# GBATZOLIS/conditional_score_diffusion

Measured on AMD Instinct MI355X. Metric: images/sec for 1000-step PC sampling, ddpm_paired_SR3 score net of celebA_SR3_160 (BASELINE configs[1]), 160x160, higher is better.
Workload: dtype f16x3 (every operand carried as hi + lo fp16 = 22 significand bits, 3 MFMAs per product, f32 accumulate; f32-class: the per-op test tolerance is the f32 kernel's, network error 1.9e-6 vs the reference); 1 GPU; BASELINE configs[1]: celebA_SR3_160 (ddpm_paired_SR3, nf=96, ch_mult (1,1,2,2,3,3), attn 20/10/5), 1000-step PC (reverse_diffusion + langevin, snr 0.15), batch 64 per GPU, random-init weights, synthetic LR inputs; images_per_gpu=64, global_batch=64, noise=on-device Philox4x32-10, precision_mode=fp16x3

## Files before the change

### conditional_score_diffusion_amd/csrc/conv_pw16.hip

```cpp
#include <stdlib.h>
#include <string.h>

#include "common.h"

namespace csd {

typedef _Float16 half8_t __attribute__((ext_vector_type(8)));
typedef float floatx4 __attribute__((ext_vector_type(4)));
typedef float v4f_t __attribute__((ext_vector_type(4)));
typedef unsigned int uint4_t __attribute__((ext_vector_type(4)));

#define PW_THREADS 256
#define PW_NTL 6
#define PW_WSCALE 256.0f
#ifndef PW_DEPTH
#define PW_DEPTH 2
#endif

struct PwKArgs {
  ConvArgs a;
  int C0, C1, Cout;
  int npix;
  int hw;
  int ks;
  int ntiles;
};

__device__ __forceinline__ float4 pw_gload4(const float* p) {
  const v4f_t v = *(const __attribute__((address_space(1))) v4f_t*)(p);
  return make_float4(v.x, v.y, v.z, v.w);
}

template <int NS, int MTP, int OCC>
__global__ __launch_bounds__(PW_THREADS, OCC) void pw16_kernel(const float* __restrict__ g_src0,
                                                          const float* __restrict__ g_src1,
                                                          const char* __restrict__ g_wpack, const PwKArgs k) {
  extern __shared__ __attribute__((aligned(16))) char smem[];
  constexpr int WPIX = MTP * 16;
  constexpr int TPIX = 4 * WPIX;
  const int tid = threadIdx.x;
  const int lane = tid & 63;
  const int wave = tid >> 6;
  const int l16 = lane & 15;
  const int kq = lane >> 4;
  const int ng = blockIdx.y;
  const int Cin = k.C0 + k.C1;

  const int wbytes = k.ks * PW_NTL * NS * 1024;
  float* const lds_bias = reinterpret_cast<float*>(smem + wbytes);
  const int col_base = ng * (PW_NTL * 16) + kq * 4;

  const int nt_mine = (k.ntiles - (int)blockIdx.x + (int)gridDim.x - 1) / (int)gridDim.x;
  const int total = nt_mine * k.ks;
  const bool has_norm = k.a.nscale != nullptr;
  const bool has_res = k.a.res != nullptr;
  const bool has_act = k.a.act == CSD_ACT_SWISH;
  const int ntl = min(PW_NTL, (k.Cout - (int)blockIdx.y * (PW_NTL * 16) + 15) / 16);

  constexpr int D = MTP == 1 ? 4 : PW_DEPTH;
  float4 raw[D][MTP][2];
  constexpr bool PFN = MTP == 1;
  float4 nsc[PFN ? D : 1][MTP][2], nsh[PFN ? D : 1][MTP][2];
  floatx4 acc[MTP][PW_NTL];
#pragma unroll
  for (int j = 0; j < MTP; ++j)
#pragma unroll
    for (int nt = 0; nt < PW_NTL; ++nt) acc[j][nt] = floatx4{0.f, 0.f, 0.f, 0.f};

  int l_tile = blockIdx.x, l_kk = 0, l_it = 0;
  int c_tile = blockIdx.x, c_kk = 0;

  auto issue = [&](float4 (&dst)[MTP][2], float4 (&dsc)[MTP][2], float4 (&dsh)[MTP][2]) {
    if (l_it < total) {
      const int kb = l_kk * 32;
      const bool s1 = kb >= k.C0;
      const float* src = s1 ? g_src1 : g_src0;
      const int C = s1 ? k.C1 : k.C0;
      const int ch = (s1 ? kb - k.C0 : kb) + kq * 8;
#pragma unroll
      for (int j = 0; j < MTP; ++j) {
        int p = l_tile * TPIX + wave * WPIX + j * 16 + l16;
        p = p < k.npix ? p : k.npix - 1;
        const float* q = src + (size_t)p * C + ch;
        dst[j][0] = pw_gload4(q);
        dst[j][1] = pw_gload4(q + 4);
        if (PFN && has_norm) {
          const size_t row = (size_t)(p / k.hw) * Cin + l_kk * 32 + kq * 8;
          dsc[j][0] = pw_gload4(k.a.nscale + row); dsc[j][1] = pw_gload4(k.a.nscale + row + 4);
          dsh[j][0] = pw_gload4(k.a.nshift + row); dsh[j][1] = pw_gload4(k.a.nshift + row + 4);
        }
      }
      ++l_it;
      if (++l_kk == k.ks) { l_kk = 0; l_tile += gridDim.x; }
    }
  };

#pragma unroll
  for (int u = 0; u < D; ++u) issue(raw[u], nsc[PFN ? u : 0], nsh[PFN ? u : 0]);

  wg_copy_to_lds<PW_THREADS, 9>(smem, g_wpack + (size_t)ng * wbytes, wbytes, tid);
  if (tid < PW_NTL * 16) {
    const int c = ng * (PW_NTL * 16) + tid;
    lds_bias[tid] = (k.a.bias && c < k.Cout) ? k.a.bias[c] : 0.f;
  }
  __syncthreads();

  for (int it = 0; it < total; it += D) {
#pragma unroll
    for (int u = 0; u < D; ++u) {
      if (it + u < total) {
        half8_t bh[MTP], bl[MTP];
#pragma unroll
        for (int j = 0; j < MTP; ++j) {
          float v[8] = {raw[u][j][0].x, raw[u][j][0].y, raw[u][j][0].z, raw[u][j][0].w,
                        raw[u][j][1].x, raw[u][j][1].y, raw[u][j][1].z, raw[u][j][1].w};
          if (has_norm) {
            float4 s0, s1, h0, h1;
            if constexpr (PFN) {
              s0 = nsc[u][j][0]; s1 = nsc[u][j][1]; h0 = nsh[u][j][0]; h1 = nsh[u][j][1];
            } else {
              int p = c_tile * TPIX + wave * WPIX + j * 16 + l16;
              p = p < k.npix ? p : k.npix - 1;
              const size_t row = (size_t)(p / k.hw) * Cin + c_kk * 32 + kq * 8;
              s0 = pw_gload4(k.a.nscale + row); s1 = pw_gload4(k.a.nscale + row + 4);
              h0 = pw_gload4(k.a.nshift + row); h1 = pw_gload4(k.a.nshift + row + 4);
            }
            const float sc[8] = {s0.x, s0.y, s0.z, s0.w, s1.x, s1.y, s1.z, s1.w};
            const float sh[8] = {h0.x, h0.y, h0.z, h0.w, h1.x, h1.y, h1.z, h1.w};
#pragma unroll
            for (int q = 0; q < 8; ++q) v[q] = fmaf(v[q], sc[q], sh[q]);
            if (has_act) {
#pragma unroll
              for (int q = 0; q < 8; ++q) v[q] = v[q] * __builtin_amdgcn_rcpf(1.0f + __expf(-v[q]));
            }
          }
#pragma unroll
          for (int q = 0; q < 8; ++q) {
            const _Float16 hi = (_Float16)v[q];
            bh[j][q] = hi;
            if (NS == 2) bl[j][q] = (_Float16)(v[q] - (float)hi);
          }
        }
        issue(raw[u], nsc[PFN ? u : 0], nsh[PFN ? u : 0]);
        const char* wk = smem + (size_t)c_kk * PW_NTL * NS * 1024 + lane * 16;
#pragma unroll
        for (int nt = 0; nt < PW_NTL; ++nt) {
          if (nt >= ntl) continue;
          const half8_t wh = *reinterpret_cast<const half8_t*>(wk + (nt * NS) * 1024);
          half8_t wl;
          if (NS == 2) wl = *reinterpret_cast<const half8_t*>(wk + (nt * NS + 1) * 1024);
#pragma unroll
          for (int j = 0; j < MTP; ++j) {
            if (NS == 2) {
              acc[j][nt] = __builtin_amdgcn_mfma_f32_16x16x32_f16(wl, bh[j], acc[j][nt], 0, 0, 0);
              acc[j][nt] = __builtin_amdgcn_mfma_f32_16x16x32_f16(wh, bl[j], acc[j][nt], 0, 0, 0);
            }
            acc[j][nt] = __builtin_amdgcn_mfma_f32_16x16x32_f16(wh, bh[j], acc[j][nt], 0, 0, 0);
          }
        }
        if (++c_kk == k.ks) {
          constexpr unsigned OOB = 0x80000000u;
          constexpr int RSRC_FLAGS = 0x00020000;
          const size_t p_base = (size_t)c_tile * TPIX + wave * WPIX;
          const int left = k.npix - (int)p_base;
          const __amdgpu_buffer_rsrc_t out_r = __builtin_amdgcn_make_buffer_rsrc(
              k.a.out + p_base * k.a.out_stride + k.a.out_coff, 0, OOB, RSRC_FLAGS);
          const __amdgpu_buffer_rsrc_t res_r = __builtin_amdgcn_make_buffer_rsrc(
              const_cast<float*>(has_res ? k.a.res + p_base * k.Cout : k.a.out), 0, OOB, RSRC_FLAGS);
          const float unscale = 1.0f / PW_WSCALE;
#pragma unroll
          for (int j = 0; j < MTP; ++j) {
            const int pl = j * 16 + l16;
            const bool pv = pl < left;
            uint4_t rv[PW_NTL];
#pragma unroll
            for (int nt = 0; nt < PW_NTL; ++nt) {
              const int col0 = col_base + nt * 16;
              const unsigned off = (pv && has_res && col0 < k.Cout) ? (unsigned)(pl * k.Cout + col0) * 4u : OOB;
              rv[nt] = __builtin_amdgcn_raw_buffer_load_b128(res_r, off, 0, 0);
            }
#pragma unroll
            for (int nt = 0; nt < PW_NTL; ++nt) {
              const int col0 = col_base + nt * 16;
              const float4 b = *reinterpret_cast<const float4*>(lds_bias + nt * 16 + kq * 4);
              uint4_t ov;
              ov.x = __float_as_uint(((acc[j][nt][0] * unscale + b.x) + __uint_as_float(rv[nt].x)) * k.a.out_scale);
              ov.y = __float_as_uint(((acc[j][nt][1] * unscale + b.y) + __uint_as_float(rv[nt].y)) * k.a.out_scale);
              ov.z = __float_as_uint(((acc[j][nt][2] * unscale + b.z) + __uint_as_float(rv[nt].z)) * k.a.out_scale);
              ov.w = __float_as_uint(((acc[j][nt][3] * unscale + b.w) + __uint_as_float(rv[nt].w)) * k.a.out_scale);
              const unsigned off = (pv && col0 < k.Cout) ? (unsigned)(pl * k.a.out_stride + col0) * 4u : OOB;
              __builtin_amdgcn_raw_buffer_store_b128(ov, out_r, off, 0, 0);
              acc[j][nt] = floatx4{0.f, 0.f, 0.f, 0.f};
            }
          }
          c_kk = 0;
          c_tile += gridDim.x;
        }
      }
    }
  }
}

static size_t pw16_w_bytes(const ConvPlan& p, int ns) { return (size_t)((p.C0 + p.C1) / 32) * PW_NTL * ns * 1024; }
static size_t pw16_lds_bytes(const ConvPlan& p, int ns) { return pw16_w_bytes(p, ns) + PW_NTL * 16 * sizeof(float); }

bool pw16_supported(const ConvPlan& p, int ns) {
  return p.taps == 1 && p.stride == 1 && p.up == 0 && p.C0 > 0 && p.C0 % 32 == 0 && p.C1 % 32 == 0 && p.Cout % 4 == 0 &&
         (ns == 1 || ns == 2) && pw16_lds_bytes(p, ns) <= 150 * 1024;
}

size_t pw16_packed_bytes(const ConvPlan& p, int ns) {
  const int n_groups = cdiv(p.Cout, PW_NTL * 16);
  return (size_t)n_groups * pw16_w_bytes(p, ns);
}

__global__ void pw16_pack_kernel(const float* __restrict__ w, _Float16* __restrict__ wpack, int layout, int cin_src,
                                 int cout_src, int cout_off, int ks, int ns, int cout_pad) {
  const size_t idx = (size_t)blockIdx.x * blockDim.x + threadIdx.x;
  const int cin_tot = ks * 32;
  const int t_lo = cout_off / 16, t_hi = (cout_off + cout_src + 15) / 16;
  if (idx >= (size_t)(t_hi - t_lo) * 16 * cin_tot) return;
  const int cp = t_lo * 16 + (int)(idx / cin_tot);
  const int cin = (int)(idx % cin_tot);
  const int cout = cp - cout_off;
  if (cp >= cout_pad || cout < 0 || cout >= cout_src || cin >= cin_src) return;
  const float v = ((layout == 0) ? w[(size_t)cout * cin_src + cin] : w[(size_t)cin * cout_src + cout]) * PW_WSCALE;
  const int ng = cp / (PW_NTL * 16), nt = (cp % (PW_NTL * 16)) / 16, r = cp % 16;
  const int kk = cin / 32, kq = (cin % 32) / 8, q = cin % 8;
  const int lane = kq * 16 + r;
  _Float16* dst = wpack + ((((size_t)ng * ks + kk) * PW_NTL + nt) * ns) * 512 + lane * 8 + q;
  const _Float16 hi = (_Float16)v;
  dst[0] = hi;
  if (ns == 2) dst[512] = (_Float16)(v - (float)hi);
}

// ... 77 lines not shown
  const int y = ty0 + ty, x = tx0 + tx;
  if (y >= H || x >= W) return;
  float acc[CO];
#pragma unroll
  for (int c = 0; c < CO; ++c) acc[c] = 0.f;
#pragma unroll
  for (int tap = 0; tap < 9; ++tap) {
    const float* q = ts_tile + ((ty + tap / 3) * 18 + tx + tap % 3) * cp + tap * CO;
#pragma unroll
    for (int c = 0; c < CO; ++c) acc[c] += q[c];
  }
#pragma unroll
  for (int c = 0; c < CO; ++c) {
    const float r = ((acc[c] + bias[c]) + (res ? res[((b * H + y) * W + x) * CO + c] : 0.f)) * out_scale;
    if (nchw) out[((b * CO + c) * H + y) * W + x] = r;
    else out[((b * H + y) * W + x) * CO + c] = r;
  }
}

int tapsum_launch(const float* part, const float* bias, const float* res, float* out, int B, int H, int W, int cout, int nchw,
                  float out_scale, hipStream_t s) {
  const int cp = pw16_taps_cout(cout);
  const dim3 grid(cdiv(W, 16), cdiv(H, 16), B), block(256);
  const size_t lds = (size_t)324 * cp * sizeof(float);
  switch (cout) {
#define CSD_TS_CASE(CO)                                                                                                              \
  case CO: {                                                                                                                         \
    static bool attr_set = false;                                                                                                    \
    if (!attr_set && lds > 64 * 1024) {                               \
      CSD_CHECK_HIP(hipFuncSetAttribute(reinterpret_cast<const void*>(tapsum_kernel<CO>), hipFuncAttributeMaxDynamicSharedMemorySize, \
                                        160 * 1024));                                                                               \
      attr_set = true;                                                                                                               \
    }                                                                                                                                \
    hipLaunchKernelGGL(tapsum_kernel<CO>, grid, block, lds, s, part, bias, res, out, H, W, cp, nchw, out_scale);                     \
    break;                                                                                                                           \
  }
    CSD_TS_CASE(1) CSD_TS_CASE(2) CSD_TS_CASE(3) CSD_TS_CASE(4) CSD_TS_CASE(5) CSD_TS_CASE(6)
#undef CSD_TS_CASE
    default:
      set_error("tapsum: %d output channels not instantiated", cout);
      return CSD_ERR_INVALID;
  }
  CSD_LAUNCH_CHECK();
  return CSD_OK;
}

bool pw16_taps_supported(int cin, int cout, int ns) {
  ConvPlan p;
  memset(&p, 0, sizeof(p));
  p.taps = 1; p.stride = 1; p.C0 = cin; p.Cout = pw16_taps_cout(cout);
  return cout >= 1 && cout <= 6 && pw16_supported(p, ns) && !CSD_TUNE_ENV("CSD_NO_TAPSUM");
}

template <int NS, int MTP, int OCC>
static int pw16_launch_t(const PwKArgs& k, const ConvPlan& p, hipStream_t s) {
  auto kern = pw16_kernel<NS, MTP, OCC>;
  const size_t lds = pw16_lds_bytes(p, NS);
  static size_t attr_lds = 0;
  if (lds > attr_lds) {
    if (hipFuncSetAttribute(reinterpret_cast<const void*>(kern), hipFuncAttributeMaxDynamicSharedMemorySize, 160 * 1024) !=
        hipSuccess) {
      set_error("pw16: cannot raise the dynamic LDS limit");
      return CSD_ERR_HIP;
    }
    attr_lds = 160 * 1024;
  }
  const int n_groups = cdiv(p.Cout, PW_NTL * 16);
  int gx = (OCC * 256) / n_groups;
  if (gx < 1) gx = 1;
  if (gx > k.ntiles) gx = k.ntiles;
  hipLaunchKernelGGL(kern, dim3(gx, n_groups), dim3(PW_THREADS), lds, s, k.a.src0, k.a.src1,
                     reinterpret_cast<const char*>(k.a.wpack), k);
  CSD_LAUNCH_CHECK();
  return CSD_OK;
}

int pw16_launch(const ConvPlan& p, int ns, const ConvArgs& a, hipStream_t s) {
  CSD_REQUIRE(pw16_supported(p, ns), "pw16: unsupported layer (taps %d C0 %d C1 %d Cout %d)", p.taps, p.C0, p.C1, p.Cout);
  CSD_REQUIRE(!a.temb && !a.out_nchw && (a.act == CSD_ACT_NONE || (a.act == CSD_ACT_SWISH && a.nscale)),
              "pw16: temb / NCHW output / an activation without a GroupNorm are not supported");
  PwKArgs k;
  k.a = a;
  k.C0 = p.C0; k.C1 = p.C1; k.Cout = p.Cout;
  k.npix = p.B * p.OH * p.OW;
  k.hw = p.OH * p.OW;
  k.ks = (p.C0 + p.C1) / 32;
  const bool big = cdiv(k.npix, 128) >= 768;
  k.ntiles = cdiv(k.npix, big ? 128 : 64);
  if (ns == 2) return big ? pw16_launch_t<2, 2, 2>(k, p, s) : pw16_launch_t<2, 1, 2>(k, p, s);
  return big ? pw16_launch_t<1, 2, 3>(k, p, s) : pw16_launch_t<1, 1, 2>(k, p, s);
}

}
```

### conditional_score_diffusion_amd/csrc/conv_f16_q.hip

```cpp
#include <stdlib.h>
#include <type_traits>

#include "conv_f16_kernel.h"

namespace csd {

typedef float floatx4q __attribute__((ext_vector_type(4)));
typedef unsigned int uint4q __attribute__((ext_vector_type(4)));

#define C16Q_THREADS 256

__device__ __forceinline__ double dpp_row16_sum(double v) {
#define CSD_DPP_STEP(CTRL)                                                                                   \
  {                                                                                                          \
    const int lo = __builtin_amdgcn_mov_dpp(__double2loint(v), CTRL, 0xF, 0xF, true);                        \
    const int hi = __builtin_amdgcn_mov_dpp(__double2hiint(v), CTRL, 0xF, 0xF, true);                        \
    v += __hiloint2double(hi, lo);                                                                           \
  }
  CSD_DPP_STEP(0xB1)
  CSD_DPP_STEP(0x4E)
  CSD_DPP_STEP(0x124)
  CSD_DPP_STEP(0x128)
#undef CSD_DPP_STEP
  return v;
}
__device__ __forceinline__ float dpp_row16_sum(float v) {
#define CSD_DPP_STEP_F(CTRL) v += __int_as_float(__builtin_amdgcn_mov_dpp(__float_as_int(v), CTRL, 0xF, 0xF, true));
  CSD_DPP_STEP_F(0xB1)
  CSD_DPP_STEP_F(0x4E)
  CSD_DPP_STEP_F(0x124)
  CSD_DPP_STEP_F(0x128)
#undef CSD_DPP_STEP_F
  return v;
}

typedef int int8q __attribute__((ext_vector_type(8)));

template <int MQ, int NS, bool MASK, int PWC, int S, int NTQ, bool F8, bool UP4 = false, bool RAW = false>
__global__ __launch_bounds__(C16Q_THREADS, 2) void conv_f16_q_kernel(const void* __restrict__ g_hi,
                                                                    const void* __restrict__ g_lo,
                                                                    const char* __restrict__ g_wpack,
                                                                    const Conv16KArgs k) {
  static_assert(!UP4 || (S == 1 && !F8), "the phase form is the stride-1 Upsample conv (a resampling conv: full split)");
  static_assert(!RAW || (NS == 2 && !F8), "the fp32-source form splits into two fp16 planes");
  constexpr int TAPS = UP4 ? 4 : 9, KS = UP4 ? 2 : 3, KCS = 2;
  constexpr int LO = 32 * KCS;
  constexpr int PSB = 32 * KCS * NS + 16;
  constexpr int NPIX = 2 * MQ * 16;
  constexpr int SPP = 2 * NS * KCS;
  constexpr int NU0 = (S == 2) ? ((NS == 2) ? 10 : 5) : ((NS == 2) ? 7 : 4);
  constexpr int NU = RAW ? 2 * ((NU0 + 1) / 2) : NU0;
  constexpr int rstride = PWC * PSB;
  constexpr int WSTEP = NTQ * NS * 1024;
  constexpr int GC = 32 * NTQ, HC = 16 * NTQ;
  extern __shared__ __attribute__((aligned(16))) char smem16[];

  const int tid = threadIdx.x;
#ifdef CSD_C16_TIMING
  int ts_n = 0;
#define Q_TSTAMP() do { if (k.a.dbg && tid == 0 && blockIdx.x < 4095 && ts_n < 8) k.a.dbg[blockIdx.x * 8 + ts_n++] = clock64(); } while (0)
#else
#define Q_TSTAMP() do { } while (0)
#endif
  Q_TSTAMP();
  const int lane = tid & 63;
  const int wave = __builtin_amdgcn_readfirstlane(tid >> 6);
  const int mi = wave >> 1, ni = wave & 1;
  const int l16 = lane & 15, kq = lane >> 4;

  int w;
  {
    const int bid = blockIdx.x, nb = k.nblocks;
    const int xcd = bid & 7, slot = bid >> 3;
    const int q = nb >> 3, r = nb & 7;
    w = (xcd < r ? xcd * (q + 1) : r * (q + 1) + (xcd - r) * q) + slot;
  }
  const int ng = w % k.n_groups;
  const int tile4 = w / k.n_groups;
  const int ph = UP4 ? (tile4 & 3) : 0, pa = ph >> 1, pb = ph & 1;
  const int tile = UP4 ? (tile4 >> 2) : tile4;
  const int tile_y = tile / k.tiles_x;
  const int ov0 = tile_y * k.TH, ox0 = (tile - tile_y * k.tiles_x) * k.TW;
  const int Py = UP4 ? 1 - pa : ((S == 2) ? 0 : 1), Px = UP4 ? 1 - pb : ((S == 2) ? 0 : 1);
  const int prow0 = ov0 * S - Py, pcol0 = ox0 * S - Px;
  const int EH = (S == 2) ? k.IH : k.OH, EW = (S == 2) ? k.IW : k.OW;
  const int Cin = k.C0;
  const int npatch = k.PH * k.PW;
// ... 515 lines not shown
    CSD_CHECK_HIP(hipFuncSetAttribute(reinterpret_cast<const void*>(kern), hipFuncAttributeMaxDynamicSharedMemorySize, 160 * 1024));
    attr_set = true;
  }
  hipLaunchKernelGGL(kern, dim3(k.nblocks), dim3(C16Q_THREADS), lds, s, static_cast<const void*>(k.a.src0),
                     static_cast<const void*>(k.a.src1), reinterpret_cast<const char*>(k.a.wpack), k);
  CSD_LAUNCH_CHECK();
  return CSD_OK;
}

template <int MQ, int NS, bool MASK, int PWC, int S, int NTQ, bool UP4>
static int launch_q_src(bool raw, const Conv16KArgs& k, size_t lds, hipStream_t s) {
  if constexpr (NS == 2 && NTQ >= 3) {
    if (raw) return launch_q<MQ, NS, MASK, PWC, S, NTQ, false, UP4, true>(k, lds, s);
  }
  if (raw) {
    set_error("conv16q: no fp32-source kernel for ns=%d NT=%d", NS, NTQ);
    return CSD_ERR_INVALID;
  }
  return launch_q<MQ, NS, MASK, PWC, S, NTQ, false, UP4, false>(k, lds, s);
}

int conv16q_launch(const ConvPlan& p, int ns, const ConvArgs& a, hipStream_t s, bool raw) {
  const bool up4 = p.up == 2;
  CSD_REQUIRE(up4 ? conv16q_up4_supported(p, ns) : conv16q_supported(p, ns), "conv16q: unsupported layer");
  CSD_REQUIRE(!a.out_nchw && a.nscale == nullptr && a.out_stride % 4 == 0 && a.out_coff % 4 == 0,
              "conv16q: NHWC fp32 output with 16-byte aligned rows, pre-normalised fp16 source");
  Conv16KArgs k;
  k.a = a;
  k.a.dbg = nullptr;
#ifdef CSD_C16_TIMING
  {
    extern long long* g_c16_dbg; extern int g_c16_dbg_blocks, g_c16_dbg_max, g_c16_dbg_n;
    const int nb = cdiv(p.OW, p.TW) * cdiv(p.B * p.OH, p.TH) * p.n_groups;
    if (g_c16_dbg && nb == g_c16_dbg_blocks && g_c16_dbg_n < g_c16_dbg_max) {
      k.a.dbg = g_c16_dbg + (size_t)g_c16_dbg_n * 4096 * 8;
      if (hipMemsetAsync(k.a.dbg, 0, 4096 * 8 * 8, s) != hipSuccess) return -1;
      long long hdr[4] = {p.C0, p.Cout, 1, (a.res ? 1 : 0) | (a.temb ? 2 : 0)};
      if (hipMemcpyAsync(k.a.dbg + 4095 * 8, hdr, sizeof(hdr), hipMemcpyHostToDevice, s) != hipSuccess) return -1;
      g_c16_dbg_n++;
    }
  }
#endif
  k.B = p.B; k.IH = p.IH; k.IW = p.IW; k.OH = p.OH; k.OW = p.OW;
  k.C0 = p.C0; k.C1 = 0; k.Cout = p.Cout;
  k.stride = p.stride; k.pad = p.stride == 2 ? 0 : 1; k.up = p.up;
  k.TH = p.TH; k.TW = p.TW; k.PH = p.PH; k.PW = p.PW;
  k.tiles_x = p.tiles_x; k.n_groups = p.n_groups;
  k.nblocks = p.tiles_x * p.tiles_y * p.n_groups * (up4 ? 4 : 1);
  if (up4) { k.OH = p.IH; k.OW = p.IW; k.up = 0; }
  k.nck = p.C0 / C16_KC;
  k.nw = 4;
  k.ntiles_n = p.Cout / 32;
  const bool mask = ((up4 ? p.IH : p.OH) % p.TH) != 0;
#define CSD_QU_CASE(MQ_, NS_, NTQ_)                                                              \
  if (up4 && p.MT == MQ_ && ns == NS_ && p.NT == NTQ_) {                                        \
    if (p.PW <= 24) {                                                                            \
      if (mask) return launch_q_src<MQ_, NS_, true, 24, 1, NTQ_, true>(raw, k, p.lds_bytes, s);    \
      return launch_q_src<MQ_, NS_, false, 24, 1, NTQ_, true>(raw, k, p.lds_bytes, s);             \
    }                                                                                            \
    if (mask) return launch_q_src<MQ_, NS_, true, 34, 1, NTQ_, true>(raw, k, p.lds_bytes, s);      \
    return launch_q_src<MQ_, NS_, false, 34, 1, NTQ_, true>(raw, k, p.lds_bytes, s);               \
  }
  CSD_QU_CASE(4, 2, 3) CSD_QU_CASE(2, 2, 3) CSD_QU_CASE(4, 1, 3) CSD_QU_CASE(2, 1, 3)
  CSD_QU_CASE(4, 2, 4) CSD_QU_CASE(2, 2, 4) CSD_QU_CASE(4, 1, 4) CSD_QU_CASE(2, 1, 4)
#undef CSD_QU_CASE
  CSD_REQUIRE(!up4, "conv16q: no phase kernel for MQ=%d ns=%d NT=%d", p.MT, ns, p.NT);
#define CSD_Q_CASE(MQ_, NS_, NTQ_)                                                  \
  if (p.MT == MQ_ && ns == NS_ && p.NT == NTQ_ && p.stride == 1) {                  \
    if (p.PW <= 24) {                                                               \
      if (mask) return launch_q_src<MQ_, NS_, true, 24, 1, NTQ_, false>(raw, k, p.lds_bytes, s);    \
      return launch_q_src<MQ_, NS_, false, 24, 1, NTQ_, false>(raw, k, p.lds_bytes, s);             \
    }                                                                               \
    if (mask) return launch_q_src<MQ_, NS_, true, 34, 1, NTQ_, false>(raw, k, p.lds_bytes, s);      \
    return launch_q_src<MQ_, NS_, false, 34, 1, NTQ_, false>(raw, k, p.lds_bytes, s);               \
  }                                                                                 \
  if (p.MT == MQ_ && ns == NS_ && p.NT == NTQ_ && p.stride == 2) {                  \
    if (p.PW <= 24) {                                                               \
      if (mask) return launch_q_src<MQ_, NS_, true, 24, 2, NTQ_, false>(raw, k, p.lds_bytes, s);    \
      return launch_q_src<MQ_, NS_, false, 24, 2, NTQ_, false>(raw, k, p.lds_bytes, s);             \
    }                                                                               \
    if (mask) return launch_q_src<MQ_, NS_, true, 34, 2, NTQ_, false>(raw, k, p.lds_bytes, s);      \
    return launch_q_src<MQ_, NS_, false, 34, 2, NTQ_, false>(raw, k, p.lds_bytes, s);               \
  }
#define CSD_Q8_CASE(MQ_, NTQ_)                                                         \
  if (p.MT == MQ_ && ns == 3 && p.NT == NTQ_ && p.stride == 1) {                     \
    if (p.PW <= 24) {                                                                \
      if (mask) return launch_q<MQ_, 2, true, 24, 1, NTQ_, true>(k, p.lds_bytes, s);  \
      return launch_q<MQ_, 2, false, 24, 1, NTQ_, true>(k, p.lds_bytes, s);           \
    }                                                                                \
    if (mask) return launch_q<MQ_, 2, true, 34, 1, NTQ_, true>(k, p.lds_bytes, s);    \
    return launch_q<MQ_, 2, false, 34, 1, NTQ_, true>(k, p.lds_bytes, s);             \
  }                                                                                  \
  if (p.MT == MQ_ && ns == 3 && p.NT == NTQ_ && p.stride == 2) {                     \
    if (p.PW <= 24) {                                                                \
      if (mask) return launch_q<MQ_, 2, true, 24, 2, NTQ_, true>(k, p.lds_bytes, s);  \
      return launch_q<MQ_, 2, false, 24, 2, NTQ_, true>(k, p.lds_bytes, s);           \
    }                                                                                \
    if (mask) return launch_q<MQ_, 2, true, 34, 2, NTQ_, true>(k, p.lds_bytes, s);    \
    return launch_q<MQ_, 2, false, 34, 2, NTQ_, true>(k, p.lds_bytes, s);             \
  }
  CSD_REQUIRE(!(raw && ns == 3), "conv16q: the fp8-correction form reads pre-split planes");
  CSD_Q8_CASE(4, 3) CSD_Q8_CASE(2, 3) CSD_Q8_CASE(2, 1)
#undef CSD_Q8_CASE
  CSD_Q_CASE(4, 2, 3) CSD_Q_CASE(2, 2, 3) CSD_Q_CASE(4, 1, 3) CSD_Q_CASE(2, 1, 3) CSD_Q_CASE(2, 2, 1)
  CSD_Q_CASE(4, 2, 4) CSD_Q_CASE(2, 2, 4) CSD_Q_CASE(4, 1, 4) CSD_Q_CASE(2, 1, 4)
#undef CSD_Q_CASE
// ... 6 lines not shown
```

Before: 1.591 images/sec.

## Specialise pointwise conv kernel for wide-LDS and narrow-Cout layers

Templates the pointwise f16 MFMA conv kernel on wave count and N-tile count. Layers whose packed weights fill more than half of the 160 KB LDS now launch 8-wave blocks at occupancy 1, so each weight copy serves more pixels. Layers with at most 32 output channels use a 2-tile accumulator with higher occupancy. The grid size is now derived from the device CU count instead of a hardcoded 256. The trade-offs are more template instantiations and a higher register or LDS footprint per block in some variants.

```diff
diff --git a/conditional_score_diffusion_amd/csrc/conv_pw16.hip b/conditional_score_diffusion_amd/csrc/conv_pw16.hip
--- a/conditional_score_diffusion_amd/csrc/conv_pw16.hip
+++ b/conditional_score_diffusion_amd/csrc/conv_pw16.hip
@@ -10,7 +10,6 @@
 typedef float v4f_t __attribute__((ext_vector_type(4)));
 typedef unsigned int uint4_t __attribute__((ext_vector_type(4)));
 
-#define PW_THREADS 256
 #define PW_NTL 6
 #define PW_WSCALE 256.0f
 #ifndef PW_DEPTH
@@ -31,13 +30,13 @@
   return make_float4(v.x, v.y, v.z, v.w);
 }
 
-template <int NS, int MTP, int OCC>
-__global__ __launch_bounds__(PW_THREADS, OCC) void pw16_kernel(const float* __restrict__ g_src0,
-                                                          const float* __restrict__ g_src1,
-                                                          const char* __restrict__ g_wpack, const PwKArgs k) {
+template <int NS, int MTP, int OCC, int WAVES, int NTL>
+__global__ __launch_bounds__(WAVES * 64, OCC) void pw16_kernel(const float* __restrict__ g_src0,
+                                                               const float* __restrict__ g_src1,
+                                                               const char* __restrict__ g_wpack, const PwKArgs k) {
   extern __shared__ __attribute__((aligned(16))) char smem[];
   constexpr int WPIX = MTP * 16;
-  constexpr int TPIX = 4 * WPIX;
+  constexpr int TPIX = WAVES * WPIX;
   const int tid = threadIdx.x;
   const int lane = tid & 63;
   const int wave = tid >> 6;
@@ -55,17 +54,17 @@
   const bool has_norm = k.a.nscale != nullptr;
   const bool has_res = k.a.res != nullptr;
   const bool has_act = k.a.act == CSD_ACT_SWISH;
-  const int ntl = min(PW_NTL, (k.Cout - (int)blockIdx.y * (PW_NTL * 16) + 15) / 16);
+  const int ntl = min(NTL, (k.Cout - (int)blockIdx.y * (PW_NTL * 16) + 15) / 16);
 
   constexpr int D = MTP == 1 ? 4 : PW_DEPTH;
   float4 raw[D][MTP][2];
   constexpr bool PFN = MTP == 1;
   float4 nsc[PFN ? D : 1][MTP][2], nsh[PFN ? D : 1][MTP][2];
-  floatx4 acc[MTP][PW_NTL];
+  floatx4 acc[MTP][NTL];
 #pragma unroll
   for (int j = 0; j < MTP; ++j)
 #pragma unroll
-    for (int nt = 0; nt < PW_NTL; ++nt) acc[j][nt] = floatx4{0.f, 0.f, 0.f, 0.f};
+    for (int nt = 0; nt < NTL; ++nt) acc[j][nt] = floatx4{0.f, 0.f, 0.f, 0.f};
 
   int l_tile = blockIdx.x, l_kk = 0, l_it = 0;
   int c_tile = blockIdx.x, c_kk = 0;
@@ -98,7 +97,7 @@
 #pragma unroll
   for (int u = 0; u < D; ++u) issue(raw[u], nsc[PFN ? u : 0], nsh[PFN ? u : 0]);
 
-  wg_copy_to_lds<PW_THREADS, 9>(smem, g_wpack + (size_t)ng * wbytes, wbytes, tid);
+  wg_copy_to_lds<WAVES * 64, 9>(smem, g_wpack + (size_t)ng * wbytes, wbytes, tid);
   if (tid < PW_NTL * 16) {
     const int c = ng * (PW_NTL * 16) + tid;
     lds_bias[tid] = (k.a.bias && c < k.Cout) ? k.a.bias[c] : 0.f;
@@ -144,7 +143,7 @@
         issue(raw[u], nsc[PFN ? u : 0], nsh[PFN ? u : 0]);
         const char* wk = smem + (size_t)c_kk * PW_NTL * NS * 1024 + lane * 16;
 #pragma unroll
-        for (int nt = 0; nt < PW_NTL; ++nt) {
+        for (int nt = 0; nt < NTL; ++nt) {
           if (nt >= ntl) continue;
           const half8_t wh = *reinterpret_cast<const half8_t*>(wk + (nt * NS) * 1024);
           half8_t wl;
@@ -172,15 +171,15 @@
           for (int j = 0; j < MTP; ++j) {
             const int pl = j * 16 + l16;
             const bool pv = pl < left;
-            uint4_t rv[PW_NTL];
-#pragma unroll
-            for (int nt = 0; nt < PW_NTL; ++nt) {
+            uint4_t rv[NTL];
+#pragma unroll
+            for (int nt = 0; nt < NTL; ++nt) {
               const int col0 = col_base + nt * 16;
               const unsigned off = (pv && has_res && col0 < k.Cout) ? (unsigned)(pl * k.Cout + col0) * 4u : OOB;
               rv[nt] = __builtin_amdgcn_raw_buffer_load_b128(res_r, off, 0, 0);
             }
 #pragma unroll
-            for (int nt = 0; nt < PW_NTL; ++nt) {
+            for (int nt = 0; nt < NTL; ++nt) {
               const int col0 = col_base + nt * 16;
               const float4 b = *reinterpret_cast<const float4*>(lds_bias + nt * 16 + kq * 4);
               uint4_t ov;
@@ -364,24 +363,17 @@
   return cout >= 1 && cout <= 6 && pw16_supported(p, ns) && !CSD_TUNE_ENV("CSD_NO_TAPSUM");
 }
 
-template <int NS, int MTP, int OCC>
-static int pw16_launch_t(const PwKArgs& k, const ConvPlan& p, hipStream_t s) {
-  auto kern = pw16_kernel<NS, MTP, OCC>;
+template <int NS, int MTP, int OCC, int WAVES, int NTL>
+static int pw16_launch_t(PwKArgs& k, const ConvPlan& p, hipStream_t s) {
+  auto kern = pw16_kernel<NS, MTP, OCC, WAVES, NTL>;
   const size_t lds = pw16_lds_bytes(p, NS);
-  static size_t attr_lds = 0;
-  if (lds > attr_lds) {
-    if (hipFuncSetAttribute(reinterpret_cast<const void*>(kern), hipFuncAttributeMaxDynamicSharedMemorySize, 160 * 1024) !=
-        hipSuccess) {
-      set_error("pw16: cannot raise the dynamic LDS limit");
-      return CSD_ERR_HIP;
-    }
-    attr_lds = 160 * 1024;
-  }
+  CSD_SET_MAX_LDS_ONCE(kern);
   const int n_groups = cdiv(p.Cout, PW_NTL * 16);
-  int gx = (OCC * 256) / n_groups;
+  k.ntiles = cdiv(k.npix, WAVES * MTP * 16);
+  int gx = (OCC * device_cu_count8()) / n_groups;
   if (gx < 1) gx = 1;
   if (gx > k.ntiles) gx = k.ntiles;
-  hipLaunchKernelGGL(kern, dim3(gx, n_groups), dim3(PW_THREADS), lds, s, k.a.src0, k.a.src1,
+  hipLaunchKernelGGL(kern, dim3(gx, n_groups), dim3(WAVES * 64), lds, s, k.a.src0, k.a.src1,
                      reinterpret_cast<const char*>(k.a.wpack), k);
   CSD_LAUNCH_CHECK();
   return CSD_OK;
@@ -398,9 +390,16 @@
   k.hw = p.OH * p.OW;
   k.ks = (p.C0 + p.C1) / 32;
   const bool big = cdiv(k.npix, 128) >= 768;
-  k.ntiles = cdiv(k.npix, big ? 128 : 64);
-  if (ns == 2) return big ? pw16_launch_t<2, 2, 2>(k, p, s) : pw16_launch_t<2, 1, 2>(k, p, s);
-  return big ? pw16_launch_t<1, 2, 3>(k, p, s) : pw16_launch_t<1, 1, 2>(k, p, s);
-}
-
-}
+  const bool wide = 2 * pw16_lds_bytes(p, ns) > 160 * 1024;
+  const bool narrow = p.Cout <= 32 && !wide;
+  if (ns == 2) {
+    if (wide) return big ? pw16_launch_t<2, 2, 1, 8, PW_NTL>(k, p, s) : pw16_launch_t<2, 1, 1, 8, PW_NTL>(k, p, s);
+    if (narrow) return big ? pw16_launch_t<2, 2, 4, 4, 2>(k, p, s) : pw16_launch_t<2, 1, 3, 4, 2>(k, p, s);
+    return big ? pw16_launch_t<2, 2, 2, 4, PW_NTL>(k, p, s) : pw16_launch_t<2, 1, 2, 4, PW_NTL>(k, p, s);
+  }
+  if (wide) return big ? pw16_launch_t<1, 2, 1, 8, PW_NTL>(k, p, s) : pw16_launch_t<1, 1, 1, 8, PW_NTL>(k, p, s);
+  if (narrow) return big ? pw16_launch_t<1, 2, 4, 4, 2>(k, p, s) : pw16_launch_t<1, 1, 3, 4, 2>(k, p, s);
+  return big ? pw16_launch_t<1, 2, 3, 4, PW_NTL>(k, p, s) : pw16_launch_t<1, 1, 2, 4, PW_NTL>(k, p, s);
+}
+
+}
```

New measurement: 1.607 images/sec (median of 6 runs). No clear change (+1.0%).

## Add persistent conv kernel for resampling convs with cross-tile prefetch

Applied to the files above, without the earlier changes.

Adds a persistent-grid variant of the fp32-source split-fp16 conv for upsample-phase and stride-2 convs. Each block walks a contiguous range of tiles, with ranges assigned per XCD. While computing the current tile it builds the next tile's index tables and prefetches that tile's first input chunk, hiding the per-tile prologue. The goal is to cut launch and tail overhead and the exposed prologue when there are more tiles than two blocks per CU. In exchange it uses more LDS for double-buffered tables, adds a large new kernel, and can be disabled through an env var.

```diff
diff --git a/conditional_score_diffusion_amd/csrc/conv_f16_q.h b/conditional_score_diffusion_amd/csrc/conv_f16_q.h
--- /dev/null
+++ b/conditional_score_diffusion_amd/csrc/conv_f16_q.h
@@ -0,0 +1,38 @@
+#pragma once
+#include "conv_f16_kernel.h"
+
+namespace csd {
+
+typedef float floatx4q __attribute__((ext_vector_type(4)));
+typedef unsigned int uint4q __attribute__((ext_vector_type(4)));
+
+#define C16Q_THREADS 256
+
+__device__ __forceinline__ double dpp_row16_sum(double v) {
+#define CSD_DPP_STEP(CTRL)                                                                                   \
+  {                                                                                                          \
+    const int lo = __builtin_amdgcn_mov_dpp(__double2loint(v), CTRL, 0xF, 0xF, true);                        \
+    const int hi = __builtin_amdgcn_mov_dpp(__double2hiint(v), CTRL, 0xF, 0xF, true);                        \
+    v += __hiloint2double(hi, lo);                                                                           \
+  }
+  CSD_DPP_STEP(0xB1)
+  CSD_DPP_STEP(0x4E)
+  CSD_DPP_STEP(0x124)
+  CSD_DPP_STEP(0x128)
+#undef CSD_DPP_STEP
+  return v;
+}
+__device__ __forceinline__ float dpp_row16_sum(float v) {
+#define CSD_DPP_STEP_F(CTRL) v += __int_as_float(__builtin_amdgcn_mov_dpp(__float_as_int(v), CTRL, 0xF, 0xF, true));
+  CSD_DPP_STEP_F(0xB1)
+  CSD_DPP_STEP_F(0x4E)
+  CSD_DPP_STEP_F(0x124)
+  CSD_DPP_STEP_F(0x128)
+#undef CSD_DPP_STEP_F
+  return v;
+}
+
+bool conv16qp_wanted(const ConvPlan& p, int ns, bool raw);
+int conv16qp_launch(const ConvPlan& p, const Conv16KArgs& k, bool mask, hipStream_t s);
+
+}
diff --git a/conditional_score_diffusion_amd/csrc/conv_f16_q.hip b/conditional_score_diffusion_amd/csrc/conv_f16_q.hip
--- a/conditional_score_diffusion_amd/csrc/conv_f16_q.hip
+++ b/conditional_score_diffusion_amd/csrc/conv_f16_q.hip
@@ -1,38 +1,9 @@
 #include <stdlib.h>
 #include <type_traits>
 
-#include "conv_f16_kernel.h"
+#include "conv_f16_q.h"
 
 namespace csd {
-
-typedef float floatx4q __attribute__((ext_vector_type(4)));
-typedef unsigned int uint4q __attribute__((ext_vector_type(4)));
-
-#define C16Q_THREADS 256
-
-__device__ __forceinline__ double dpp_row16_sum(double v) {
-#define CSD_DPP_STEP(CTRL)                                                                                   \
-  {                                                                                                          \
-    const int lo = __builtin_amdgcn_mov_dpp(__double2loint(v), CTRL, 0xF, 0xF, true);                        \
-    const int hi = __builtin_amdgcn_mov_dpp(__double2hiint(v), CTRL, 0xF, 0xF, true);                        \
-    v += __hiloint2double(hi, lo);                                                                           \
-  }
-  CSD_DPP_STEP(0xB1)
-  CSD_DPP_STEP(0x4E)
-  CSD_DPP_STEP(0x124)
-  CSD_DPP_STEP(0x128)
-#undef CSD_DPP_STEP
-  return v;
-}
-__device__ __forceinline__ float dpp_row16_sum(float v) {
-#define CSD_DPP_STEP_F(CTRL) v += __int_as_float(__builtin_amdgcn_mov_dpp(__float_as_int(v), CTRL, 0xF, 0xF, true));
-  CSD_DPP_STEP_F(0xB1)
-  CSD_DPP_STEP_F(0x4E)
-  CSD_DPP_STEP_F(0x124)
-  CSD_DPP_STEP_F(0x128)
-#undef CSD_DPP_STEP_F
-  return v;
-}
 
 typedef int int8q __attribute__((ext_vector_type(8)));
 
@@ -654,6 +625,7 @@
   k.nw = 4;
   k.ntiles_n = p.Cout / 32;
   const bool mask = ((up4 ? p.IH : p.OH) % p.TH) != 0;
+  if (conv16qp_wanted(p, ns, raw)) return conv16qp_launch(p, k, mask, s);
 #define CSD_QU_CASE(MQ_, NS_, NTQ_)                                                              \
   if (up4 && p.MT == MQ_ && ns == NS_ && p.NT == NTQ_) {                                        \
     if (p.PW <= 24) {                                                                            \
diff --git a/conditional_score_diffusion_amd/csrc/conv_f16_qp.hip b/conditional_score_diffusion_amd/csrc/conv_f16_qp.hip
--- /dev/null
+++ b/conditional_score_diffusion_amd/csrc/conv_f16_qp.hip
@@ -0,0 +1,389 @@
+#include <stdlib.h>
+#include <atomic>
+#include <type_traits>
+
+#include "conv_f16_q.h"
+
+namespace csd {
+
+template <int MQ, bool MASK, int PWC, int S, int NTQ, bool UP4>
+__global__ __launch_bounds__(C16Q_THREADS, 2) void conv_f16_qp_kernel(const float* __restrict__ g_src,
+                                                                     const char* __restrict__ g_wpack,
+                                                                     const Conv16KArgs k, const int nitems) {
+  static_assert(!UP4 || S == 1, "the phase form is the stride-1 Upsample conv");
+  constexpr int NS = 2, NP = 2;
+  constexpr int TAPS = UP4 ? 4 : 9, KS = UP4 ? 2 : 3, KCS = 2;
+  constexpr int LO = 32 * KCS;
+  constexpr int PSB = 32 * KCS * NS + 16;
+  constexpr int NPIX = 2 * MQ * 16;
+  constexpr int NU0 = (S == 2) ? 10 : 7;
+  constexpr int NU = 2 * ((NU0 + 1) / 2);
+  constexpr int rstride = PWC * PSB;
+  constexpr int WSTEP = NTQ * NS * 1024;
+  constexpr int GC = 32 * NTQ, HC = 16 * NTQ;
+  constexpr int BR = UP4 ? 2 : 3;
+  static_assert(TAPS % BR == 0, "weight ring phase");
+  extern __shared__ __attribute__((aligned(16))) char smem16[];
+
+  const int tid = threadIdx.x;
+  const int lane = tid & 63;
+  const int wave = __builtin_amdgcn_readfirstlane(tid >> 6);
+  const int mi = wave >> 1, ni = wave & 1;
+  const int l16 = lane & 15, kq = lane >> 4;
+
+  int it0, it1;
+  {
+    const int bid = blockIdx.x, nb = gridDim.x;
+    const int xcd = bid & 7, slot = bid >> 3;
+    const int q = nb >> 3, r = nb & 7;
+    const int v = (xcd < r ? xcd * (q + 1) : r * (q + 1) + (xcd - r) * q) + slot;
+    it0 = (int)((long long)v * nitems / nb);
+    it1 = (int)((long long)(v + 1) * nitems / nb);
+  }
+  if (it0 >= it1) return;
+
+  const int EH = (S == 2) ? k.IH : k.OH, EW = (S == 2) ? k.IW : k.OW;
+  const int Cin = k.C0;
+  const int npatch = k.PH * k.PW;
+  const int patch_bytes = k.PH * PWC * PSB;
+  const int tabsz = 3 * NPIX + npatch;
+  int* const dtab = reinterpret_cast<int*>(smem16 + patch_bytes);
+  int* const tab0 = dtab + npatch;
+
+  struct Item { int ng, tile4, pa, pb, ov0, ox0; };
+  auto item_of = [&](int w) -> Item {
+    Item it;
+    it.ng = w % k.n_groups;
+    it.tile4 = w / k.n_groups;
+    const int ph = UP4 ? (it.tile4 & 3) : 0;
+    it.pa = ph >> 1; it.pb = ph & 1;
+    const int tile = UP4 ? (it.tile4 >> 2) : it.tile4;
+    const int tile_y = tile / k.tiles_x;
+    it.ov0 = tile_y * k.TH;
+    it.ox0 = (tile - tile_y * k.tiles_x) * k.TW;
+    return it;
+  };
+  auto build_tables = [&](int* tab, const Item& it) {
+    int* const otab = tab; int* const btab = otab + NPIX; int* const vtab = btab + NPIX; int* const stab = vtab + NPIX;
+    const int ov0 = it.ov0, ox0 = it.ox0;
+    const int Py = UP4 ? 1 - it.pa : ((S == 2) ? 0 : 1), Px = UP4 ? 1 - it.pb : ((S == 2) ? 0 : 1);
+    const int prow0 = ov0 * S - Py, pcol0 = ox0 * S - Px;
+    for (int m = tid; m < NPIX; m += C16Q_THREADS) {
+      const int ty = m / k.TW, tx = m - ty * k.TW;
+      const int ov = ov0 + ty, ox = ox0 + tx;
+      const bool mv = (m < k.TH * k.TW) && (ov < k.B * k.OH) && (ox < k.OW);
+      const int b = ov / k.OH, oy = ov - b * k.OH;
+      unsigned vb = 0;
+#pragma unroll
+      for (int r = 0; r < KS; ++r) {
+        const int iy = oy * S + r - Py, ix = ox * S + r - Px;
+        vb |= ((mv && iy >= 0 && iy < EH) ? 1u : 0u) << r;
+        vb |= ((mv && ix >= 0 && ix < EW) ? 1u : 0u) << (3 + r);
+      }
+      otab[m] = mv ? (UP4 ? (ov - ov0) * 4 * k.OW + 2 * ox : (ov - ov0) * k.OW + ox) : -1;
+      btab[m] = mv ? b : 0;
+      vtab[m] = (int)vb;
+    }
+    for (int pix = tid; pix < npatch; pix += C16Q_THREADS) {
+      const int pr = pix / k.PW, pc = pix - pr * k.PW;
+      const int vr = prow0 + pr, col = pcol0 + pc;
+      const int img_lo = MASK ? 0 : (ov0 / k.OH) * EH;
+      const int img_hi = MASK ? k.B * EH : img_lo + EH;
+      const bool in = vr >= img_lo && vr < img_hi && col >= 0 && col < EW;
+      const int sb = vr / EH, sr = vr - sb * EH;
+      stab[pix] = in ? (sb * k.IH + sr) * k.IW + col : -1;
+    }
+  };
+
+  const int total4 = npatch * 2 * KCS;
+  auto raw_load = [&](const int* stab, int e, int cb, int half) -> float4 {
+    float4 v = make_float4(0.f, 0.f, 0.f, 0.f);
+    if (e < total4) {
+      const int pix = e / (2 * KCS), grp = e - pix * (2 * KCS);
+      const int sp = stab[pix];
+      if (sp >= 0) v = gload4f(g_src + (size_t)sp * Cin + cb + grp * 8 + half * 4);
+    }
+    return v;
+  };
+  auto raw_store = [&](int e, const float4& a, const float4& b) {
+    if (e >= total4) return;
+    const int pix = e / (2 * KCS), grp = e - pix * (2 * KCS);
+    const float v[8] = {a.x, a.y, a.z, a.w, b.x, b.y, b.z, b.w};
+    half8 h, l;
+#pragma unroll
+    for (int j = 0; j < 8; ++j) {
+      h[j] = (_Float16)v[j];
+      l[j] = (_Float16)(v[j] - (float)h[j]);
+    }
+    *reinterpret_cast<half8*>(smem16 + dtab[pix] + grp * 16) = h;
+    *reinterpret_cast<half8*>(smem16 + dtab[pix] + LO + grp * 16) = l;
+  };
+
+  for (int pix = tid; pix < npatch; pix += C16Q_THREADS) {
+    const int pr = pix / k.PW, pc = pix - pr * k.PW;
+    dtab[pix] = (pr * PWC + pc) * PSB;
+  }
+  Item cur = item_of(it0);
+  build_tables(tab0, cur);
+  int base[MQ];
+#pragma unroll
+  for (int j = 0; j < MQ; ++j) {
+    const int m = (mi * MQ + j) * 16 + l16;
+    const int ty = m / k.TW, tx = m - ty * k.TW;
+    base[j] = (m < k.TH * k.TW) ? ty * S * rstride + tx * S * PSB + kq * 16 : kq * 16;
+  }
+  __syncthreads();
+  {
+    float4 v0[NU];
+#pragma unroll
+    for (int j = 0; j < NU; ++j) v0[j] = raw_load(tab0 + 3 * NPIX, (j >> 1) * C16Q_THREADS + tid, 0, j & 1);
+#pragma unroll
+    for (int j = 0; j < NU; j += 2) raw_store((j >> 1) * C16Q_THREADS + tid, v0[j], v0[j + 1]);
+  }
+  __syncthreads();
+
+  const int nk32 = Cin / 32;
+  const int nstage = nk32;
+  constexpr unsigned OOB = 0x80000000u;
+  constexpr int RSRC_FLAGS = 0x00020000;
+  const float wunscale = 1.0f / C16_WSCALE;
+  const bool has_res = k.a.res != nullptr, has_temb = k.a.temb != nullptr;
+
+  int set = 0;
+  for (int w = it0; w < it1; ++w) {
+    const bool has_next = w + 1 < it1;
+    int* const otab = tab0 + set * tabsz;
+    int* const btab = otab + NPIX;
+    int* const vtab = btab + NPIX;
+    int* const stab = vtab + NPIX;
+    int* const ntab = tab0 + (set ^ 1) * tabsz;
+    const Item nxt = item_of(has_next ? w + 1 : w);
+    const int ph = cur.pa * 2 + cur.pb;
+
+    unsigned vbits[MQ];
+    if (MASK) {
+#pragma unroll
+      for (int j = 0; j < MQ; ++j) vbits[j] = (unsigned)vtab[(mi * MQ + j) * 16 + l16];
+    }
+    const char* wstep = g_wpack + ((size_t)((UP4 ? ph * k.n_groups * 2 : 0) + cur.ng * 2 + ni) * nk32 * TAPS) * WSTEP + lane * 16;
+    half8 wreg[BR][NTQ][NP];
+#pragma unroll
+    for (int q = 0; q < BR - 1; ++q)
+#pragma unroll
+      for (int t = 0; t < NTQ; ++t)
+#pragma unroll
+        for (int p = 0; p < NP; ++p) wreg[q][t][p] = gload_h8(wstep + (size_t)q * WSTEP + (t * NS + p) * 1024);
+    wstep += (size_t)(BR - 2) * WSTEP;
+
+    floatx4q acc[MQ][NTQ];
+#pragma unroll
+    for (int j = 0; j < MQ; ++j)
+#pragma unroll
+      for (int t = 0; t < NTQ; ++t) acc[j][t] = floatx4q{0.f, 0.f, 0.f, 0.f};
+
+    for (int stg = 0; stg < nstage; ++stg) {
+      const bool more = stg + 1 < nstage;
+      const bool fetch = more || has_next;
+      float4 sv[NU];
+      if (fetch) {
+        const int* const st_ = more ? stab : ntab + 3 * NPIX;
+        const int cb = more ? (stg + 1) * 32 : 0;
+#pragma unroll
+        for (int j = 0; j < NU; ++j) sv[j] = raw_load(st_, (j >> 1) * C16Q_THREADS + tid, cb, j & 1);
+      }
+      if (stg == 0 && has_next) build_tables(ntab, nxt);
+      constexpr int RING = 2;
+      half8 preg[RING][NP];
+      auto load_frag = [&](int q) {
+        const int tap_ = q / MQ, j_ = q % MQ;
+        const char* p = smem16 + base[j_] + (tap_ / KS) * rstride + (tap_ % KS) * PSB;
+#pragma unroll
+        for (int pl = 0; pl < NP; ++pl) preg[q % RING][pl] = *reinterpret_cast<const half8*>(p + pl * LO);
+      };
+#pragma unroll
+      for (int q = 0; q < RING - 1; ++q) load_frag(q);
+#pragma unroll
+      for (int tap = 0; tap < TAPS; ++tap) {
+        const int bc = tap % BR, bn = (tap + BR - 1) % BR;
+        const int r = tap / KS, sx = tap % KS;
+        wstep += WSTEP;
+#pragma unroll
+        for (int t = 0; t < NTQ; ++t)
+#pragma unroll
+          for (int p = 0; p < NP; ++p) wreg[bn][t][p] = gload_h8(wstep + (t * NS + p) * 1024);
+#pragma unroll
+        for (int j = 0; j < MQ; ++j) {
+          const int q = tap * MQ + j;
+          if (q + RING - 1 < TAPS * MQ) load_frag(q + RING - 1);
+          __builtin_amdgcn_sched_barrier(0);
+          half8 b[NP];
+          const bool v = !MASK || (((vbits[j] >> r) & 1u) && ((vbits[j] >> (3 + sx)) & 1u));
+#pragma unroll
+          for (int pl = 0; pl < NP; ++pl) {
+            b[pl] = preg[q % RING][pl];
+            if (MASK && !v) {
+#pragma unroll
+              for (int e = 0; e < 8; ++e) b[pl][e] = (_Float16)0.f;
+            }
+          }
+#pragma unroll
+          for (int t = 0; t < NTQ; ++t) {
+            acc[j][t] = __builtin_amdgcn_mfma_f32_16x16x32_f16(wreg[bc][t][1], b[0], acc[j][t], 0, 0, 0);
+            acc[j][t] = __builtin_amdgcn_mfma_f32_16x16x32_f16(wreg[bc][t][0], b[1], acc[j][t], 0, 0, 0);
+            acc[j][t] = __builtin_amdgcn_mfma_f32_16x16x32_f16(wreg[bc][t][0], b[0], acc[j][t], 0, 0, 0);
+          }
+          __builtin_amdgcn_sched_barrier(0);
+        }
+      }
+      if (fetch) {
+        __syncthreads();
+#pragma unroll
+        for (int j = 0; j < NU; j += 2) raw_store((j >> 1) * C16Q_THREADS + tid, sv[j], sv[j + 1]);
+        if (more) __syncthreads();
+      }
+    }
+
+    const int ov0 = cur.ov0, pa = cur.pa, pb = cur.pb, ng = cur.ng, tile4 = cur.tile4;
+    const size_t o_base = UP4 ? ((size_t)(2 * ov0 + pa) * 2 * k.OW + pb) : (size_t)ov0 * k.OW;
+    const int b0 = ov0 / k.OH;
+    const __amdgpu_buffer_rsrc_t out_r =
+        __builtin_amdgcn_make_buffer_rsrc(k.a.out + o_base * k.a.out_stride + k.a.out_coff, 0, OOB, RSRC_FLAGS);
+    const __amdgpu_buffer_rsrc_t res_r = __builtin_amdgcn_make_buffer_rsrc(
+        const_cast<float*>(has_res ? k.a.res + o_base * k.Cout : k.a.out), 0, OOB, RSRC_FLAGS);
+    const int c_base = ng * GC + ni * HC + kq * 4;
+    int oidx[MQ];
+#pragma unroll
+    for (int j = 0; j < MQ; ++j) oidx[j] = otab[(mi * MQ + j) * 16 + l16];
+    float4 bias4[NTQ], tvu4[NTQ];
+#pragma unroll
+    for (int t = 0; t < NTQ; ++t) {
+      const int c0 = c_base + t * 16;
+      bias4[t] = k.a.bias ? gload4f(k.a.bias + c0) : make_float4(0.f, 0.f, 0.f, 0.f);
+      tvu4[t] = (!MASK && has_temb) ? gload4f(k.a.temb + (size_t)b0 * k.a.temb_stride + c0) : make_float4(0.f, 0.f, 0.f, 0.f);
+    }
+    float4 addv[MQ][NTQ];
+#pragma unroll
+    for (int j = 0; j < MQ; ++j)
+#pragma unroll
+      for (int t = 0; t < NTQ; ++t) {
+        float4 a = tvu4[t];
+        if (has_res) {
+          const unsigned off = oidx[j] >= 0 ? (unsigned)(oidx[j] * k.Cout + c_base + t * 16) * 4u : OOB;
+          const uint4q rv = __builtin_amdgcn_raw_buffer_load_b128(res_r, off, 0, 0);
+          const float4 rr = make_float4(__uint_as_float(rv.x), __uint_as_float(rv.y), __uint_as_float(rv.z), __uint_as_float(rv.w));
+          a = (MASK || !has_temb) ? rr : make_float4(rr.x + a.x, rr.y + a.y, rr.z + a.z, rr.w + a.w);
+        }
+        addv[j][t] = a;
+      }
+    if (MASK && has_temb) {
+#pragma unroll
+      for (int j = 0; j < MQ; ++j) {
+        const int b = btab[(mi * MQ + j) * 16 + l16];
+#pragma unroll
+        for (int t = 0; t < NTQ; ++t) {
+          const float4 tv = gload4f(k.a.temb + (size_t)b * k.a.temb_stride + c_base + t * 16);
+          addv[j][t] = make_float4(addv[j][t].x + tv.x, addv[j][t].y + tv.y, addv[j][t].z + tv.z, addv[j][t].w + tv.w);
+        }
+      }
+    }
+    using st_t = typename std::conditional<UP4, float, double>::type;
+    st_t st_s[NTQ][4], st_q[NTQ][4];
+#pragma unroll
+    for (int t = 0; t < NTQ; ++t)
+#pragma unroll
+      for (int i = 0; i < 4; ++i) { st_s[t][i] = 0; st_q[t][i] = 0; }
+#pragma unroll
+    for (int j = 0; j < MQ; ++j)
+#pragma unroll
+      for (int t = 0; t < NTQ; ++t) {
+        const float b4[4] = {bias4[t].x, bias4[t].y, bias4[t].z, bias4[t].w};
+        const float a4[4] = {addv[j][t].x, addv[j][t].y, addv[j][t].z, addv[j][t].w};
+        float o4[4];
+#pragma unroll
+        for (int i = 0; i < 4; ++i) {
+          o4[i] = ((acc[j][t][i] * wunscale + b4[i]) + a4[i]) * k.a.out_scale;
+          const st_t dv = oidx[j] >= 0 ? (st_t)o4[i] : (st_t)0;
+          st_s[t][i] += dv;
+          st_q[t][i] = fma(dv, dv, st_q[t][i]);
+        }
+        uint4q ov;
+        ov.x = __float_as_uint(o4[0]); ov.y = __float_as_uint(o4[1]); ov.z = __float_as_uint(o4[2]); ov.w = __float_as_uint(o4[3]);
+        const unsigned off = oidx[j] >= 0 ? (unsigned)(oidx[j] * k.a.out_stride + c_base + t * 16) * 4u : OOB;
+        __builtin_amdgcn_raw_buffer_store_b128(ov, out_r, off, 0, 0);
+      }
+    if (k.a.stats) {
+#pragma unroll
+      for (int t = 0; t < NTQ; ++t)
+#pragma unroll
+        for (int i = 0; i < 4; ++i) {
+          const double s = (double)dpp_row16_sum(st_s[t][i]), q = (double)dpp_row16_sum(st_q[t][i]);
+          if (l16 == 0)
+            *reinterpret_cast<double2*>(k.a.stats + (((size_t)tile4 * 2 + mi) * k.Cout + c_base + t * 16 + i) * 2) = make_double2(s, q);
+        }
+    }
+    if (!has_next) break;
+    __syncthreads();
+    cur = nxt;
+    set ^= 1;
+  }
+}
+
+static std::atomic<long long> g_qp_launches[4], g_qp_oneshot{0};
+
+static size_t qp_lds_bytes(const ConvPlan& p) { return p.lds_bytes + ((size_t)3 * 2 * p.MT * 16 + (size_t)p.PH * p.PW) * sizeof(int); }
+static int qp_grid() { return 2 * device_cu_count8(); }
+
+bool conv16qp_wanted(const ConvPlan& p, int ns, bool raw) {
+  const bool form = raw && ns == 2 && (p.up == 2 || (p.stride == 2 && p.up == 0)) && p.NT == 3 && (p.MT == 2 || p.MT == 4) &&
+                    p.C0 >= 64 && 2 * qp_lds_bytes(p) <= (size_t)160 * 1024;
+  if (!form) return false;
+  const long nitems = (long)p.tiles_x * p.tiles_y * p.n_groups * (p.up == 2 ? 4 : 1);
+  const bool yes = nitems > qp_grid() && !CSD_TUNE_ENV("CSD_NO_QP");
+  if (!yes) g_qp_oneshot++;
+  return yes;
+}
+
+template <int MQ, bool MASK, int PWC, int S, int NTQ, bool UP4>
+static int launch_qp(const Conv16KArgs& k, size_t lds, hipStream_t s) {
+  auto kern = conv_f16_qp_kernel<MQ, MASK, PWC, S, NTQ, UP4>;
+  CSD_SET_MAX_LDS_ONCE(kern);
+  const int nitems = k.nblocks;
+  const int grid = nitems < qp_grid() ? nitems : qp_grid();
+  hipLaunchKernelGGL(kern, dim3(grid), dim3(C16Q_THREADS), lds, s, k.a.src0, reinterpret_cast<const char*>(k.a.wpack), k, nitems);
+  CSD_LAUNCH_CHECK();
+  g_qp_launches[(UP4 ? 2 : 0) + (MASK ? 1 : 0)]++;
+  return CSD_OK;
+}
+
+template <int MQ, int NTQ>
+static int pick_qp(const ConvPlan& p, const Conv16KArgs& k, bool mask, size_t lds, hipStream_t s) {
+#define CSD_QP_FORM(S_, UP4_)                                                         \
+  {                                                                                   \
+    if (p.PW <= 24) {                                                                 \
+      if (mask) return launch_qp<MQ, true, 24, S_, NTQ, UP4_>(k, lds, s);             \
+      return launch_qp<MQ, false, 24, S_, NTQ, UP4_>(k, lds, s);                      \
+    }                                                                                 \
+    if (mask) return launch_qp<MQ, true, 34, S_, NTQ, UP4_>(k, lds, s);               \
+    return launch_qp<MQ, false, 34, S_, NTQ, UP4_>(k, lds, s);                        \
+  }
+  if (p.up == 2) CSD_QP_FORM(1, true)
+  CSD_QP_FORM(2, false)
+#undef CSD_QP_FORM
+}
+
+int conv16qp_launch(const ConvPlan& p, const Conv16KArgs& k, bool mask, hipStream_t s) {
+  const size_t lds = qp_lds_bytes(p);
+  if (p.MT == 4 && p.NT == 3) return pick_qp<4, 3>(p, k, mask, lds, s);
+  if (p.MT == 2 && p.NT == 3) return pick_qp<2, 3>(p, k, mask, lds, s);
+  set_error("conv16qp: no kernel for MQ=%d NT=%d", p.MT, p.NT);
+  return CSD_ERR_INVALID;
+}
+
+}
+
+extern "C" int csd_debug_resample_schedule(long long out[5]) {
+  if (!out) return CSD_ERR_INVALID;
+  for (int i = 0; i < 4; ++i) out[i] = csd::g_qp_launches[i].load();
+  out[4] = csd::g_qp_oneshot.load();
+  return CSD_OK;
+}
```

After: 1.621 images/sec before, 1.613 images/sec after. No clear change (-0.5%).
